# facebookresearch/fast3r

Measured on AMD Instinct MI355X. Metric: views/sec (512^2, ViT-L) single forward pass at N=320, higher is better.
Workload: dtype fp16

## Files before the change

fast3r_amd/csrc/f3r_common.h:

```cpp
#pragma once
#include <hip/hip_runtime.h>
#include <stdint.h>

#include "../../include/f3r.h"

typedef uint32_t u32x4 __attribute__((ext_vector_type(4)));
typedef uint32_t u32x2 __attribute__((ext_vector_type(2)));
typedef _Float16 half8 __attribute__((ext_vector_type(8)));
typedef __bf16 bf8 __attribute__((ext_vector_type(8)));
typedef float float4v __attribute__((ext_vector_type(4)));
typedef float float16v __attribute__((ext_vector_type(16)));

struct F16 {
  typedef _Float16 elem;
  typedef half8 vec8;
  static constexpr int id = F3R_F16;
  static __device__ __forceinline__ float4v mfma16(vec8 a, vec8 b, float4v c) {
    return __builtin_amdgcn_mfma_f32_16x16x32_f16(a, b, c, 0, 0, 0);
  }
  static __device__ __forceinline__ float16v mfma32(vec8 a, vec8 b, float16v c) {
    return __builtin_amdgcn_mfma_f32_32x32x16_f16(a, b, c, 0, 0, 0);
  }
  static __device__ __forceinline__ float16v mfma32k8(u32x2 a, u32x2 b, float16v c) {
    typedef _Float16 h4 __attribute__((ext_vector_type(4)));
    return __builtin_amdgcn_mfma_f32_32x32x8f16(__builtin_bit_cast(h4, a), __builtin_bit_cast(h4, b), c, 0, 0, 0);
  }
  static __device__ __forceinline__ float sum2(uint32_t pk, float acc) {
    typedef _Float16 h2 __attribute__((ext_vector_type(2)));
    const h2 ones = {(_Float16)1.0f, (_Float16)1.0f};
    return __builtin_amdgcn_fdot2(__builtin_bit_cast(h2, pk), ones, acc, false);
  }
};
struct BF16 {
  typedef __bf16 elem;
  typedef bf8 vec8;
  static constexpr int id = F3R_BF16;
  static __device__ __forceinline__ float4v mfma16(vec8 a, vec8 b, float4v c) {
    return __builtin_amdgcn_mfma_f32_16x16x32_bf16(a, b, c, 0, 0, 0);
  }
  static __device__ __forceinline__ float16v mfma32(vec8 a, vec8 b, float16v c) {
    return __builtin_amdgcn_mfma_f32_32x32x16_bf16(a, b, c, 0, 0, 0);
  }
  static __device__ __forceinline__ float16v mfma32k8(u32x2 a, u32x2 b, float16v c) {
    typedef short s4 __attribute__((ext_vector_type(4)));
    return __builtin_amdgcn_mfma_f32_32x32x8bf16_1k(__builtin_bit_cast(s4, a), __builtin_bit_cast(s4, b), c, 0, 0, 0);
  }
  static __device__ __forceinline__ float sum2(uint32_t pk, float acc) {
    typedef __bf16 b2 __attribute__((ext_vector_type(2)));
    const b2 ones = {(__bf16)1.0f, (__bf16)1.0f};
    return __builtin_amdgcn_fdot2_f32_bf16(__builtin_bit_cast(b2, pk), ones, acc, false);
  }
};

template <class T>
__device__ __forceinline__ uint16_t to_lp(float x) {
  typename T::elem e = (typename T::elem)x;
  return __builtin_bit_cast(uint16_t, e);
}
template <class T>
__device__ __forceinline__ uint32_t pack2(float lo, float hi) {
  typedef typename T::elem e2 __attribute__((ext_vector_type(2)));
  e2 p;
  p[0] = (typename T::elem)lo;
  p[1] = (typename T::elem)hi;
  return __builtin_bit_cast(uint32_t, p);
}
template <class T>
__device__ __forceinline__ float from_lp(uint16_t b) {
  return (float)__builtin_bit_cast(typename T::elem, b);
}
template <class T>
__device__ __forceinline__ float lo_f(uint32_t w) { return from_lp<T>((uint16_t)(w & 0xffffu)); }
template <class T>
__device__ __forceinline__ float hi_f(uint32_t w) { return from_lp<T>((uint16_t)(w >> 16)); }

__device__ __forceinline__ uint32_t relu_pk(uint32_t w) {
  uint32_t neg = (w >> 15) & 0x00010001u;
  return w & ~(neg * 0xffffu);
}

template <class T>
__device__ __forceinline__ typename T::vec8 as_vec8(u32x4 v) {
  return __builtin_bit_cast(typename T::vec8, v);
}

bool f3r_gemm256_eligible(const f3r_gemm_args& a);
bool f3r_gemm256_preferred(const f3r_gemm_args& a);
int f3r_gemm256_launch(const f3r_gemm_args& a, hipStream_t stream, int stagger);
int f3r_gemm256_lab(const f3r_gemm_args& a, hipStream_t stream);

bool f3r_gemm_asm_eligible(const f3r_gemm_args& a, const char** why);
bool f3r_gemm_asm_preferred(int64_t tiles);
int f3r_gemm_asm_launch(const f3r_gemm_args& a, hipStream_t stream);
bool f3r_gemm_asm_f8_eligible(const f3r_gemm_args& a, const char** why);
int f3r_gemm_asm_f8_launch(const f3r_gemm_args& a, hipStream_t stream);
bool f3r_gemm_asm_qkv_eligible(const f3r_gemm_args& a, const char** why);
int f3r_gemm_asm_qkv_launch(const f3r_gemm_args& a, hipStream_t stream);

bool f3r_attn_asm_eligible(const f3r_attn_args& a, int64_t min_keys, const char** why);
int f3r_attn_asm_launch(const f3r_attn_args& a, hipStream_t stream);
bool f3r_attn_asm_uses_q256(const f3r_attn_args& a);
bool f3r_attn_asm_splits_tail(const f3r_attn_args& a);

int f3r_attn_generic_launch(const f3r_attn_args& a, hipStream_t stream);

void f3r_set_error(const char* fmt, ...);
int f3r_check_launch(const char* what);

#define F3R_REQUIRE(cond, ...)        \
  do {                                \
    if (!(cond)) {                    \
      f3r_set_error(__VA_ARGS__);     \
      return F3R_ERR_ARG;             \
    }                                 \
  } while (0)
```

fast3r_amd/csrc/f3r_gemm.hip:

```cpp
#include <stdlib.h>

#include "f3r_common.h"
#include "f3r_gemm_epi.h"

namespace {

constexpr int BM = 128, BN = 128, BK = 64, NT = 256;
constexpr int TILE_ELEMS = 128 * 64;
constexpr int GEMM_LDS_BYTES = 2 * 2 * TILE_ELEMS * 2;

__device__ __forceinline__ int swz(int row, int chunk) { return row * 64 + ((chunk ^ ((row >> 1) & 7)) << 3); }

struct ConvRow {
  int b, oy, ox;
  bool ok;
};

template <class T, int A_MODE, int EPI, int GLDS>
__global__ __launch_bounds__(NT, 2) void gemm_kernel(const f3r_gemm_args p) {
  extern __shared__ __attribute__((aligned(16))) uint16_t smem[];
  uint16_t* As = smem;
  uint16_t* Ws = smem + 2 * TILE_ELEMS;

  const int tid = threadIdx.x;
  const int lane = tid & 63;
  const int wid = __builtin_amdgcn_readfirstlane(tid >> 6);
  const int wm = wid >> 1, wn = wid & 1;

  const int n_tiles_n = (p.N + BN - 1) / BN;
  const int64_t n_tiles_m = (p.M + BM - 1) / BM;
  const int64_t n_wg = n_tiles_m * n_tiles_n;
  int64_t wg = blockIdx.x;
  {
    const int64_t q = n_wg / 8, r = n_wg % 8;
    const int64_t xcd = wg % 8, idx = wg / 8;
    wg = (xcd < r ? xcd * (q + 1) : r * (q + 1) + (xcd - r) * q) + idx;
  }
  constexpr int GM = 8;
  const int64_t per_group = (int64_t)GM * n_tiles_n;
  const int64_t grp = wg / per_group;
  const int64_t first_m = grp * GM;
  const int gm = (int)((n_tiles_m - first_m) < GM ? (n_tiles_m - first_m) : GM);
  const int64_t rem_ = wg - grp * per_group;
  const int tn = (int)(rem_ / gm);
  const int64_t tm = first_m + rem_ % gm;
  const int64_t m0 = tm * BM;
  const int n0 = tn * BN;

  const int sc = tid & 7;
  const int sr0 = tid >> 3;
  const uint16_t* Ag = (const uint16_t*)p.A;
  const uint16_t* Wg = (const uint16_t*)p.W;

  ConvRow cr[4];
  int64_t a_row_off[4];
  bool a_row_ok[4];
  bool w_row_ok[4];
  int64_t w_row_off[4];
#pragma unroll
  for (int i = 0; i < 4; ++i) {
    const int64_t m = m0 + sr0 + 32 * i;
    a_row_ok[i] = m < p.M;
    if (A_MODE == F3R_A_PLAIN) {
      a_row_off[i] = m * p.lda;
    } else {
      const int64_t per_img = (int64_t)p.conv_OH * p.conv_OW;
      const int64_t mm = a_row_ok[i] ? m : 0;
      cr[i].b = (int)(mm / per_img);
      const int rem = (int)(mm % per_img);
      cr[i].oy = rem / p.conv_OW;
      cr[i].ox = rem % p.conv_OW;
      cr[i].ok = a_row_ok[i];
      a_row_off[i] = 0;
    }
    const int n = n0 + sr0 + 32 * i;
    w_row_ok[i] = n < p.N;
    w_row_off[i] = (int64_t)n * p.Kpad;
  }

  const int nseg = p.split == F3R_SPLIT_NONE ? 1 : (p.split == F3R_SPLIT_W2 ? 2 : 3);
  const int Kpad1 = p.split == F3R_SPLIT_NONE ? p.Kpad : p.Kpad / 2;
  const int nk1 = Kpad1 / BK;
  const int nk = nseg * nk1;
  const int cpad_tiles = (A_MODE == F3R_A_CONV3X3) ? ((p.conv_C + 63) / 64) : 1;
  const uint16_t* Alo = (const uint16_t*)p.A_lo;

  u32x4 ra[4], rw[4];
  auto load_tile = [&](int kt_all) {
    const int seg = kt_all / nk1;
    const int kt = kt_all - seg * nk1;
    const uint16_t* Ag = (seg == 2) ? Alo : (const uint16_t*)p.A;
    if (A_MODE == F3R_A_PLAIN) {
      const int k = kt * BK + sc * 8;
      const bool kok = (k + 8) <= p.K;
#pragma unroll
      for (int i = 0; i < 4; ++i) {
        u32x4 v = {0u, 0u, 0u, 0u};
        if (a_row_ok[i] && kok) v = *(const u32x4*)(Ag + a_row_off[i] + k);
        ra[i] = v;
      }
    } else {
      const int tap = kt / cpad_tiles;
      const int ci = (kt - tap * cpad_tiles) * 64 + sc * 8;
      const int dy = tap / 3 - 1, dx = tap % 3 - 1;
      const bool cok = ci < p.conv_C;
#pragma unroll
      for (int i = 0; i < 4; ++i) {
        const int iy = cr[i].oy * p.conv_stride + dy;
        const int ix = cr[i].ox * p.conv_stride + dx;
        u32x4 v = {0u, 0u, 0u, 0u};
        if (cr[i].ok && cok && iy >= 0 && iy < p.conv_H && ix >= 0 && ix < p.conv_W) {
          const int64_t off = (((int64_t)cr[i].b * p.conv_H + iy) * p.conv_W + ix) * p.conv_C + ci;
          v = *(const u32x4*)(Ag + off);
          if (p.a_relu) {
            v[0] = relu_pk(v[0]);
            v[1] = relu_pk(v[1]);
            v[2] = relu_pk(v[2]);
            v[3] = relu_pk(v[3]);
          }
        }
        ra[i] = v;
      }
    }
    const int kw = (seg == 1 ? Kpad1 : 0) + kt * BK + sc * 8;
#pragma unroll
    for (int i = 0; i < 4; ++i) {
      u32x4 v = {0u, 0u, 0u, 0u};
      if (w_row_ok[i]) v = *(const u32x4*)(Wg + w_row_off[i] + kw);
      rw[i] = v;
    }
  };
  auto store_tile = [&](int buf) {
    uint16_t* a = As + buf * TILE_ELEMS;
    uint16_t* w = Ws + buf * TILE_ELEMS;
#pragma unroll
    for (int i = 0; i < 4; ++i) {
      const int r = sr0 + 32 * i;
      *(u32x4*)(a + swz(r, sc)) = ra[i];
      *(u32x4*)(w + swz(r, sc)) = rw[i];
    }
  };

  float4v acc[4][4];
#pragma unroll
  for (int i = 0; i < 4; ++i)
#pragma unroll
    for (int j = 0; j < 4; ++j) acc[i][j] = float4v{0.f, 0.f, 0.f, 0.f};

  const int Dq_ = p.qkv_dq ? p.qkv_dq : p.N / 3;
  const bool swap_roles = (EPI == F3R_EPI_QKV) && (n0 + wn * 64 >= Dq_ + (p.N - Dq_) / 2);

  const int fr = lane & 15;
  const int fg = lane >> 4;

  const int offA = (swap_roles ? 0 : 2 * TILE_ELEMS);
  const int offB = (swap_roles ? 2 * TILE_ELEMS : 0);
  const int rowA = (swap_roles ? wm : wn) * 64 + fr;
  const int rowB = (swap_roles ? wn : wm) * 64 + fr;

  auto compute = [&](int buf) {
    const uint16_t* ta = smem + offA + buf * TILE_ELEMS;
    const uint16_t* tb = smem + offB + buf * TILE_ELEMS;
#pragma unroll
    for (int ks = 0; ks < 2; ++ks) {
      typename T::vec8 fa[4], fb[4];
#pragma unroll
      for (int f = 0; f < 4; ++f) {
        fa[f] = as_vec8<T>(*(const u32x4*)(ta + swz(rowA + f * 16, ks * 4 + fg)));
        fb[f] = as_vec8<T>(*(const u32x4*)(tb + swz(rowB + f * 16, ks * 4 + fg)));
      }
#pragma unroll
      for (int i = 0; i < 4; ++i)
#pragma unroll
        for (int j = 0; j < 4; ++j) acc[i][j] = T::mfma16(fa[i], fb[j], acc[i][j]);
    }
  };

  if constexpr (GLDS == 1) {
    typedef __attribute__((address_space(3))) void* lds_ptr_t;
    typedef const __attribute__((address_space(1))) void* glb_ptr_t;
    const int lrow = lane >> 3, pch = lane & 7;
    const uint16_t* asrc[4];
    const uint16_t* wsrc[4];
#pragma unroll
    for (int i = 0; i < 4; ++i) {
      const int r = (wid * 4 + i) * 8 + lrow;
      const int lch = pch ^ ((r >> 1) & 7);
      int64_t m = m0 + r;
      if (m >= p.M) m = p.M - 1;
      int n = n0 + r;
      if (n >= p.N) n = p.N - 1;
      asrc[i] = Ag + m * p.lda + lch * 8;
      wsrc[i] = Wg + (int64_t)n * p.Kpad + lch * 8;
    }
    const int64_t alo_delta = Alo ? (Alo - Ag) : 0;
    auto dma_tile = [&](int kt_all, int buf) {
      const int seg = kt_all / nk1;
      const int kt = kt_all - seg * nk1;
      const int64_t ka = (seg == 2 ? alo_delta : 0) + (int64_t)kt * BK;
      const int kw = (seg == 1 ? Kpad1 : 0) + kt * BK;
#pragma unroll
      for (int i = 0; i < 4; ++i) {
        uint16_t* la = As + buf * TILE_ELEMS + (wid * 4 + i) * 8 * 64;
        uint16_t* lw = Ws + buf * TILE_ELEMS + (wid * 4 + i) * 8 * 64;
        __builtin_amdgcn_global_load_lds((glb_ptr_t)(asrc[i] + ka), (lds_ptr_t)la, 16, 0, 0);
        __builtin_amdgcn_global_load_lds((glb_ptr_t)(wsrc[i] + kw), (lds_ptr_t)lw, 16, 0, 0);
      }
    };
    dma_tile(0, 0);
    __syncthreads();
    int cur = 0;
    for (int kt = 0; kt < nk; ++kt) {
      if (kt + 1 < nk) dma_tile(kt + 1, cur ^ 1);
      compute(cur);
      __syncthreads();
      cur ^= 1;
    }
  } else {
    load_tile(0);
    store_tile(0);
    __syncthreads();
    int cur = 0;
    for (int kt = 0; kt < nk; ++kt) {
      const bool more = (kt + 1) < nk;
      if (more) load_tile(kt + 1);
      compute(cur);
      if (more) store_tile(cur ^ 1);
      __syncthreads();
      cur ^= 1;
    }
  }

  const int64_t m_base = m0 + wm * 64;
  const int n_base = n0 + wn * 64;
  if (swap_roles) gemm_epilogue_vt<T, GemmFragLayout<4, 4, 4, 4>, true>(p, &acc[0][0], m_base, n_base, lane);
  else gemm_epilogue_default<T, EPI, GemmFragLayout<4, 4, 4, 4>, true>(p, &acc[0][0], m_base, n_base, lane);
}

template <class T, int A_MODE, int EPI, int GLDS>
int launch(const f3r_gemm_args& a, hipStream_t stream) {
  static bool attr_set = false;
  auto kern = gemm_kernel<T, A_MODE, EPI, GLDS>;
  if (!attr_set) {
    (void)hipFuncSetAttribute((const void*)kern, hipFuncAttributeMaxDynamicSharedMemorySize, GEMM_LDS_BYTES);
    attr_set = true;
  }
  const int64_t tiles = ((a.M + BM - 1) / BM) * ((a.N + BN - 1) / BN);
  if (tiles <= 0) return F3R_OK;
  F3R_REQUIRE(tiles < (1ll << 31), "f3r_gemm: grid too large");
  hipLaunchKernelGGL(kern, dim3((unsigned)tiles), dim3(NT), GEMM_LDS_BYTES, stream, a);
  return f3r_check_launch("f3r_gemm");
}

template <class T>
int dispatch(const f3r_gemm_args& a, hipStream_t stream) {
  if (a.a_mode == F3R_A_CONV3X3) return launch<T, F3R_A_CONV3X3, F3R_EPI_GENERIC, 0>(a, stream);
  const int Kpad1 = a.split ? a.Kpad / 2 : a.Kpad;
  const bool glds = a.K == Kpad1 && a.M > 0;
  switch (a.epi) {
    case F3R_EPI_GENERIC: return glds ? launch<T, F3R_A_PLAIN, F3R_EPI_GENERIC, 1>(a, stream) : launch<T, F3R_A_PLAIN, F3R_EPI_GENERIC, 0>(a, stream);
    case F3R_EPI_QKV: return glds ? launch<T, F3R_A_PLAIN, F3R_EPI_QKV, 1>(a, stream) : launch<T, F3R_A_PLAIN, F3R_EPI_QKV, 0>(a, stream);
    case F3R_EPI_CONVT: return launch<T, F3R_A_PLAIN, F3R_EPI_CONVT, 0>(a, stream);
  }
  f3r_set_error("f3r_gemm: bad epi %d", a.epi);
  return F3R_ERR_ARG;
}

inline bool al16(const void* p) { return (((uintptr_t)p) & 15) == 0; }
inline bool al8(const void* p) { return (((uintptr_t)p) & 7) == 0; }

}

extern "C" int f3r_gemm(const f3r_gemm_args* args, f3r_stream_t stream) {
  F3R_REQUIRE(args != nullptr, "f3r_gemm: null args");
  const f3r_gemm_args& a = *args;
  F3R_REQUIRE(a.A && a.W, "f3r_gemm: null operand");
  F3R_REQUIRE(a.M >= 0 && a.N > 0, "f3r_gemm: bad M/N (%lld, %d)", (long long)a.M, a.N);
  F3R_REQUIRE(a.split >= F3R_SPLIT_NONE && a.split <= F3R_SPLIT_X3F8, "f3r_gemm: bad split %d", a.split);
  if (a.split == F3R_SPLIT_W2F8) {
    F3R_REQUIRE(al16(a.A) && al16(a.W) && a.w_scale && (((uintptr_t)a.w_scale) & 3) == 0, "f3r_gemm: W2F8 needs 16-byte aligned A / W and w_scale");
    F3R_REQUIRE(a.K > 0 && a.K % 128 == 0 && a.Kpad == a.K, "f3r_gemm: W2F8 needs K = Kpad, a multiple of 128 (got %d / %d)", a.K, a.Kpad);
    F3R_REQUIRE(a.lda % 8 == 0 && a.lda * 2 >= (int64_t)a.K * 3, "f3r_gemm: W2F8 rows are [K fp16 | K fp8]: lda %lld must be >= 3 K / 2", (long long)a.lda);
    F3R_REQUIRE(a.epi != F3R_EPI_GENERIC || a.out_f32 || a.out_lp, "f3r_gemm: no output");
    F3R_REQUIRE(!a.out_f8 && !a.out_relu_f8 && !a.fin_w, "f3r_gemm: W2F8 launches write one output (no out_f8 / out_relu_f8 / fin_w)");
    F3R_REQUIRE((a.kernel_sel >= 0 && a.kernel_sel <= 7) || a.kernel_sel == 9, "f3r_gemm: bad kernel_sel %d", a.kernel_sel);
    F3R_REQUIRE(a.dtype == F3R_F16, "f3r_gemm: W2F8 corrects fp16 planes only (dtype %d)", a.dtype);
    F3R_REQUIRE(a.act >= F3R_ACT_NONE && a.act <= F3R_ACT_RELU, "f3r_gemm: bad act %d", a.act);
    F3R_REQUIRE(a.N % 4 == 0 && (!a.bias || al16(a.bias)), "f3r_gemm: N %d must be a multiple of 4, bias 16-byte aligned", a.N);
    if (a.epi == F3R_EPI_GENERIC) {
      F3R_REQUIRE(!a.out_f32 || (al16(a.out_f32) && a.ldo_f32 % 4 == 0 && a.ldo_f32 >= a.N), "f3r_gemm: out_f32 alignment/ld");
      F3R_REQUIRE(!a.out_lp || (al16(a.out_lp) && a.ldo_lp % 8 == 0 && a.ldo_lp >= a.N), "f3r_gemm: out_lp alignment/ld");
      F3R_REQUIRE(!a.res_f32 || (al16(a.res_f32) && a.ldr_f32 % 4 == 0 && a.ldr_f32 >= a.N), "f3r_gemm: res_f32 alignment/ld");
    }
    const char* why = "";
    if (a.epi == F3R_EPI_QKV) {
      F3R_REQUIRE(a.qkv_dq != 0 || a.N % 3 == 0, "f3r_gemm: QKV with three equal parts needs N %% 3 == 0 (got %d)", a.N);
      {
        const int Dq = a.qkv_dq ? a.qkv_dq : a.N / 3;
        F3R_REQUIRE(Dq > 0 && Dq % 64 == 0 && a.N > Dq && (a.N - Dq) % 128 == 0, "f3r_gemm: QKV parts must be whole 64-wide heads (N %d, q %d)", a.N, Dq);
      }
      F3R_REQUIRE(a.q && a.k && a.vt && a.W_aux && al16(a.W_aux) && a.seq_len > 0 && a.M % a.seq_len == 0 && a.ldvt >= a.seq_len && a.act == F3R_ACT_NONE,
                  "f3r_gemm: W2F8 QKV needs q, k, vt, W_aux (16-byte aligned), seq_len dividing M, no activation");
      if (a.rope_cos) F3R_REQUIRE(a.rope_sin && a.rope_w > 0 && al16(a.rope_cos) && al16(a.rope_sin), "f3r_gemm: RoPE tables");
      if (!f3r_gemm_asm_qkv_eligible(a, &why)) {
        f3r_set_error("f3r_gemm: split W2F8 QKV but the launch is not eligible for the hand-scheduled kernel: %s", why);
        return F3R_ERR_UNSUPPORTED;
      }
      return f3r_gemm_asm_qkv_launch(a, (hipStream_t)stream);
    }
    if (!f3r_gemm_asm_f8_eligible(a, &why)) {
      f3r_set_error("f3r_gemm: split W2F8 (fp8 low plane) but the launch is not eligible for the hand-scheduled kernel: %s", why);
      return F3R_ERR_UNSUPPORTED;
    }
    return f3r_gemm_asm_f8_launch(a, (hipStream_t)stream);
  }
  F3R_REQUIRE(a.epi == F3R_EPI_GENERIC || (!a.out_f8 && !a.out_relu_f8 && !a.fin_w), "f3r_gemm: out_f8 / out_relu_f8 / fin_w need the generic epilogue (epi %d)", a.epi);
  const int planes = a.split ? 2 : 1;
  F3R_REQUIRE(a.Kpad > 0 && a.Kpad % (64 * planes) == 0, "f3r_gemm: Kpad %d must be a positive multiple of %d", a.Kpad, 64 * planes);
  const int Kpad1 = a.Kpad / planes;
  F3R_REQUIRE((a.split != F3R_SPLIT_X3 && a.split != F3R_SPLIT_X3F8) || (a.A_lo && al16(a.A_lo) && !a.a_relu), "f3r_gemm: X3 / X3F8 split needs A_lo (16-byte aligned) and no a_relu");
  if (a.split == F3R_SPLIT_X3F8)
    F3R_REQUIRE(a.a_mode == F3R_A_CONV3X3 && a.dtype == F3R_F16 && a.conv_C % 128 == 0 && a.w_scale && (((uintptr_t)a.w_scale) & 3) == 0,
                "f3r_gemm: X3F8 needs a 3x3 convolution with conv_C %% 128 == 0 (got %d), fp16 planes and w_scale", a.conv_C);
  F3R_REQUIRE((a.kernel_sel >= 0 && a.kernel_sel <= 7) || a.kernel_sel == 9 || a.kernel_sel >= 16, "f3r_gemm: bad kernel_sel %d", a.kernel_sel);
  F3R_REQUIRE(a.N % 4 == 0, "f3r_gemm: N %d must be a multiple of 4", a.N);
  F3R_REQUIRE(al16(a.A) && al16(a.W), "f3r_gemm: A/W must be 16-byte aligned");
  F3R_REQUIRE(a.dtype == F3R_F16 || a.dtype == F3R_BF16, "f3r_gemm: bad dtype %d", a.dtype);
  if (a.a_mode == F3R_A_PLAIN) {
    F3R_REQUIRE(a.K > 0 && a.K % 8 == 0 && a.K <= Kpad1, "f3r_gemm: K %d must be a multiple of 8 and <= Kpad", a.K);
    F3R_REQUIRE(a.lda % 8 == 0 && a.lda >= a.K, "f3r_gemm: lda %lld must be a multiple of 8 and >= K", (long long)a.lda);
  } else if (a.a_mode == F3R_A_CONV3X3) {
    F3R_REQUIRE(a.conv_C > 0 && a.conv_C % 8 == 0, "f3r_gemm: conv_C %d must be a multiple of 8", a.conv_C);
    F3R_REQUIRE(Kpad1 == 9 * ((a.conv_C + 63) / 64) * 64, "f3r_gemm: conv Kpad %d != 9*roundup(C,64) per plane", a.Kpad);
    F3R_REQUIRE(a.epi == F3R_EPI_GENERIC, "f3r_gemm: conv3x3 supports only the generic epilogue");
    F3R_REQUIRE(a.conv_stride == 1 || a.conv_stride == 2, "f3r_gemm: conv stride %d", a.conv_stride);
    F3R_REQUIRE(a.conv_OH == (a.conv_H + 2 - 3) / a.conv_stride + 1 && a.conv_OW == (a.conv_W + 2 - 3) / a.conv_stride + 1,
                "f3r_gemm: conv output dims inconsistent");
    F3R_REQUIRE(a.conv_OH > 0 && a.conv_OW > 0 && a.M % ((int64_t)a.conv_OH * a.conv_OW) == 0, "f3r_gemm: conv M not a multiple of OH*OW");
  } else {
    f3r_set_error("f3r_gemm: bad a_mode %d", a.a_mode);
    return F3R_ERR_ARG;
  }
  if (a.epi == F3R_EPI_GENERIC) {
    F3R_REQUIRE(a.out_f32 || a.out_lp || a.fin_w, "f3r_gemm: no output");
    F3R_REQUIRE(!a.out_f32 || (al16(a.out_f32) && a.ldo_f32 % 4 == 0 && a.ldo_f32 >= a.N), "f3r_gemm: out_f32 alignment/ld");
    F3R_REQUIRE(!a.out_lp || (al8(a.out_lp) && a.ldo_lp % 4 == 0 && a.ldo_lp >= a.N), "f3r_gemm: out_lp alignment/ld");
    F3R_REQUIRE((!a.out_f8 && !a.out_relu_f8) || (a.dtype == F3R_F16 && a.N % 8 == 0 && al8(a.out_f8) && al8(a.out_relu_f8) && !a.out_lp_f8),
                "f3r_gemm: out_f8 / out_relu_f8 need fp16, N %% 8 == 0 and 8-byte aligned buffers");
    if (a.fin_w) {
      F3R_REQUIRE(a.fin_b && a.fin_pts && al16(a.fin_w) && (a.fin_n_out == 3 || a.fin_n_out == 4) && (a.fin_n_out == 4 || !a.fin_conf),
                  "f3r_gemm: fin_w needs fin_b, fin_pts, a 16-byte aligned [4][N] weight and fin_n_out 3 or 4 (a confidence output needs 4)");
      F3R_REQUIRE(a.fin_depth_mode >= 0 && a.fin_depth_mode <= 2 && (a.fin_conf_mode == 0 || a.fin_conf_mode == 1), "f3r_gemm: bad fin_depth_mode / fin_conf_mode");
      F3R_REQUIRE(!a.out_f32 && !a.out_relu && !a.out_f8 && !a.out_relu_f8 && !a.res_lp && !a.res_f32 && !a.rowadd,
                  "f3r_gemm: the fused head tail writes fin_pts / fin_conf only");
    }
    F3R_REQUIRE(!a.res_f32 || (al16(a.res_f32) && a.ldr_f32 % 4 == 0), "f3r_gemm: res_f32 alignment/ld");
    F3R_REQUIRE(!a.res_lp || (al8(a.res_lp) && a.ldr_lp % 4 == 0), "f3r_gemm: res_lp alignment/ld");
    F3R_REQUIRE(!a.res_lp2 || (al8(a.res_lp2) && a.ldr_lp2 % 4 == 0), "f3r_gemm: res_lp2 alignment/ld");
    F3R_REQUIRE((!a.res_lp_lo || (a.res_lp && al8(a.res_lp_lo))) && (!a.res_lp2_lo || (a.res_lp2 && al8(a.res_lp2_lo))), "f3r_gemm: low residual planes need their high planes");
    F3R_REQUIRE((!a.out_lp_lo || (a.out_lp && al8(a.out_lp_lo))) && (!a.out_relu || (al8(a.out_relu) && a.ldo_lp % 4 == 0 && a.ldo_lp >= a.N)) &&
                (!a.out_relu_lo || (a.out_relu && al8(a.out_relu_lo))), "f3r_gemm: out_lp_lo / out_relu alignment");
    F3R_REQUIRE(!a.rowadd || (al16(a.rowadd) && a.rowadd_div > 0), "f3r_gemm: rowadd alignment/div");
    const int64_t ld_max = 1ll << 26;
    F3R_REQUIRE((!a.out_f32 || a.ldo_f32 < ld_max) && (!a.out_lp || a.ldo_lp < ld_max) && (!a.res_f32 || (a.ldr_f32 >= 0 && a.ldr_f32 < ld_max)) &&
                (!a.res_lp || (a.ldr_lp >= 0 && a.ldr_lp < ld_max)) && (!a.res_lp2 || (a.ldr_lp2 >= 0 && a.ldr_lp2 < ld_max)), "f3r_gemm: row strides must be < 2^26 elements");
    F3R_REQUIRE(!a.bias || al16(a.bias), "f3r_gemm: bias alignment");
  } else if (a.epi == F3R_EPI_QKV) {
    const int Dq = a.qkv_dq ? a.qkv_dq : a.N / 3;
    F3R_REQUIRE(a.qkv_dq != 0 || a.N % 3 == 0, "f3r_gemm: QKV with three equal parts needs N %% 3 == 0 (got %d)", a.N);
    F3R_REQUIRE(Dq > 0 && Dq % 64 == 0 && a.N > Dq && (a.N - Dq) % 128 == 0, "f3r_gemm: QKV parts must be whole 64-wide heads (N %d, q %d)", a.N, Dq);
    F3R_REQUIRE(a.q && a.k && a.vt && al8(a.q) && al8(a.k) && al8(a.vt), "f3r_gemm: QKV outputs null/misaligned");
    F3R_REQUIRE(a.seq_len > 0 && a.M % a.seq_len == 0 && a.ldvt >= a.seq_len, "f3r_gemm: QKV seq_len/ldvt");
    F3R_REQUIRE(a.act == F3R_ACT_NONE, "f3r_gemm: QKV has no activation");
    F3R_REQUIRE(!a.bias || al16(a.bias), "f3r_gemm: bias alignment");
    if (a.rope_cos) F3R_REQUIRE(a.rope_sin && a.rope_w > 0 && al16(a.rope_cos) && al16(a.rope_sin), "f3r_gemm: RoPE tables");
  } else if (a.epi == F3R_EPI_CONVT) {
    F3R_REQUIRE(a.out_lp && al8(a.out_lp), "f3r_gemm: CONVT needs out_lp");
    F3R_REQUIRE(a.ct_s > 0 && a.ct_cout > 0 && a.ct_cout % 4 == 0 && a.N == a.ct_s * a.ct_s * a.ct_cout, "f3r_gemm: CONVT N != s*s*cout");
    F3R_REQUIRE(a.ct_h > 0 && a.ct_w > 0 && a.M % ((int64_t)a.ct_h * a.ct_w) == 0, "f3r_gemm: CONVT M not a multiple of h*w");
    F3R_REQUIRE(!a.bias || al16(a.bias), "f3r_gemm: bias alignment");
  }
  hipStream_t s = (hipStream_t)stream;
  if (a.kernel_sel >= 16) return f3r_gemm256_lab(a, s);
  if (a.split == F3R_SPLIT_X3F8 || a.fin_w) {
    if (!f3r_gemm256_eligible(a)) {
      f3r_set_error("f3r_gemm: split X3F8 / fin_w but the launch is not eligible for the 256-tile kernel (conv_C %% 64 (X3F8: 128) == 0, "
                    "N %% 128 == 0 (fin_w: N == 128), operand below 4 GiB)");
      return F3R_ERR_UNSUPPORTED;
    }
    return f3r_gemm256_launch(a, s, 1);
  }
  if (a.kernel_sel == 6 || a.kernel_sel == 0 || a.kernel_sel == 9) {
    const char* why = "";
    if (a.epi == F3R_EPI_QKV && f3r_gemm_asm_qkv_eligible(a, &why) && (a.kernel_sel == 6 || a.kernel_sel == 9 || f3r_gemm_asm_preferred((a.M / 256) * (a.N / 3 / 256))))
      return f3r_gemm_asm_qkv_launch(a, s);
    const bool ok = a.epi != F3R_EPI_QKV && f3r_gemm_asm_eligible(a, &why);
    if ((a.kernel_sel == 6 || a.kernel_sel == 9) && !ok) {
      f3r_set_error("f3r_gemm: kernel_sel 6 (hand-scheduled kernel) but the launch is not eligible: %s", why);
      return F3R_ERR_UNSUPPORTED;
    }
    if (ok && (a.kernel_sel == 6 || a.kernel_sel == 9 || f3r_gemm_asm_preferred((a.M / 256) * (a.N / 256)))) return f3r_gemm_asm_launch(a, s);
  }
  const int sel = a.kernel_sel == 7 ? 0 : a.kernel_sel;
  if (sel >= 2) F3R_REQUIRE(f3r_gemm256_eligible(a), "f3r_gemm: kernel_sel %d but the shape is not eligible for the 256-tile kernel", sel);
  if (sel >= 2 || (sel == 0 && f3r_gemm256_eligible(a) && f3r_gemm256_preferred(a))) return f3r_gemm256_launch(a, s, sel != 3);
  return a.dtype == F3R_F16 ? dispatch<F16>(a, s) : dispatch<BF16>(a, s);
}
```

fast3r_amd/csrc/f3r_gemm256.hip:

```cpp
#include "f3r_gemm256_impl.h"

int f3r_gemm256_run_bf16(const f3r_gemm_args& a, hipStream_t stream, int stagger);
int f3r_gemm256_run_conv_f8_fin(const f3r_gemm_args& a, hipStream_t stream);

bool f3r_gemm256_eligible(const f3r_gemm_args& a) {
  if (a.N % 128 != 0) return false;
  if (a.epi == F3R_EPI_QKV) {
    const int Dq = a.qkv_dq ? a.qkv_dq : a.N / 3;
    if (Dq % 256 != 0 || ((a.N - Dq) / 2) % 256 != 0) return false;
  }
  const int Kpad1 = a.split ? a.Kpad / 2 : a.Kpad;
  if (Kpad1 % 64 != 0) return false;
  if (a.a_mode == F3R_A_PLAIN) {
    if (a.K != Kpad1) return false;
    if ((int64_t)256 * a.lda * 2 >= (1ll << 32)) return false;
  } else {
    if (a.a_relu || a.conv_C % 64 != 0) return false;
    if (a.M / ((int64_t)a.conv_OH * a.conv_OW) * a.conv_H * a.conv_W * a.conv_C * 2 >= (1ll << 32)) return false;
    if (a.split == F3R_SPLIT_X3F8 && (a.conv_C % 128 != 0 || a.dtype != F3R_F16)) return false;
  }
  if (a.split == F3R_SPLIT_X3F8 && a.a_mode != F3R_A_CONV3X3) return false;
  if (a.fin_w && (a.a_mode != F3R_A_CONV3X3 || a.N != 128 || a.epi != F3R_EPI_GENERIC)) return false;
  if ((int64_t)256 * a.Kpad * 2 >= (1ll << 32)) return false;
  const int add = gemm_additive_pattern(a);
  if (add == F3R_ADD_UNSUPPORTED || (add != F3R_ADD_NONE && a.act != F3R_ACT_NONE)) return false;
  if (add != F3R_ADD_NONE && a.epi != F3R_EPI_GENERIC) return false;
  if (a.a_mode == F3R_A_CONV3X3 ? (add == F3R_ADD_RES_F32 || add == F3R_ADD_ROWADD) : add == F3R_ADD_RES_LP) return false;
  return true;
}

bool f3r_gemm256_preferred(const f3r_gemm_args& a) { return score_256(a, tile_halves(a)) >= score_128(a); }

int f3r_gemm256_launch(const f3r_gemm_args& a, hipStream_t stream, int stagger) {
  const int64_t tiles = ((a.M + BM - 1) / BM) * ((a.N + 127) / 128);
  if (tiles <= 0) return F3R_OK;
  F3R_REQUIRE(tiles < (1ll << 31), "f3r_gemm: grid too large");
  if (a.split == F3R_SPLIT_X3F8 || a.fin_w) return f3r_gemm256_run_conv_f8_fin(a, stream);
  return a.dtype == F3R_F16 ? dispatch256<F16>(a, stream, stagger) : f3r_gemm256_run_bf16(a, stream, stagger);
}
```

fast3r_amd/csrc/f3r_gemm256_f8.hip:

```cpp
#include <cstdlib>

#include "f3r_gemm256_impl.h"

int f3r_gemm256_run_conv_f8_fin(const f3r_gemm_args& a, hipStream_t stream) {
  const bool f8 = a.split == F3R_SPLIT_X3F8;
  const int add = gemm_additive_pattern(a);
  if (a.fin_w) {
#ifdef F3R_CONV_ABLATIONS
    if (f8) {
      static const char* ab = getenv("F3R_CONV_ABLATE");
      switch (ab ? atoi(ab) : 0) {
#define F3R_ABL(n) case n: return launch256<F16, F3R_A_CONV3X3, F3R_EPI_GENERIC, 1, F3R_ADD_NONE, 1, true, true, false, n>(a, stream);
        F3R_ABL(1) F3R_ABL(1024) F3R_ABL(2048) F3R_ABL(2) F3R_ABL(4) F3R_ABL(3) F3R_ABL(7)
#undef F3R_ABL
      }
    }
#endif
    if (a.dtype == F3R_BF16) return launch256<BF16, F3R_A_CONV3X3, F3R_EPI_GENERIC, 1, F3R_ADD_NONE, 1, false, true>(a, stream);
    if (f8 && a.kernel_sel == 5) return launch256<F16, F3R_A_CONV3X3, F3R_EPI_GENERIC, 1, F3R_ADD_NONE, 1, true, true, true>(a, stream);
    return f8 ? launch256<F16, F3R_A_CONV3X3, F3R_EPI_GENERIC, 1, F3R_ADD_NONE, 1, true, true>(a, stream)
              : launch256<F16, F3R_A_CONV3X3, F3R_EPI_GENERIC, 1, F3R_ADD_NONE, 1, false, true>(a, stream);
  }
  const int nh = tile_halves(a);
  if (add == F3R_ADD_RES_LP)
    return nh == 2 ? launch256<F16, F3R_A_CONV3X3, F3R_EPI_GENERIC, 1, F3R_ADD_RES_LP, 2, true>(a, stream)
                   : launch256<F16, F3R_A_CONV3X3, F3R_EPI_GENERIC, 1, F3R_ADD_RES_LP, 1, true>(a, stream);
  return nh == 2 ? launch256<F16, F3R_A_CONV3X3, F3R_EPI_GENERIC, 1, F3R_ADD_NONE, 2, true>(a, stream)
                 : launch256<F16, F3R_A_CONV3X3, F3R_EPI_GENERIC, 1, F3R_ADD_NONE, 1, true>(a, stream);
}
```

Measured before the change: 35.87.

## Add strip-staged persistent 3x3 conv kernel for X3F8 split convolutions

Adds a persistent conv kernel for the X3F8 fp16+fp8 3x3 convolution. It loads a contiguous 264-row strip of input pixels into LDS once per (dy, channel-tile) and reuses it across the three dx taps by shifting the fragment read address. Image-edge columns are handled by redirecting reads to zeroed LDS blocks rather than reloading the operand per tap. It also prefetches the next tile's operands before the epilogue. By default it is chosen when kernel_sel is 0 and the launch is the fused head tail (fin_w) or has N not a multiple of 256. This trades per-tap global/LDS traffic for more LDS, a single workgroup per CU, and extra complexity in edge masking.

```diff
diff --git a/fast3r_amd/csrc/f3r_common.h b/fast3r_amd/csrc/f3r_common.h
--- a/fast3r_amd/csrc/f3r_common.h
+++ b/fast3r_amd/csrc/f3r_common.h
@@ -86,6 +86,7 @@
 
 bool f3r_gemm256_eligible(const f3r_gemm_args& a);
 bool f3r_gemm256_preferred(const f3r_gemm_args& a);
+bool f3r_conv_strip_eligible(const f3r_gemm_args& a);
 int f3r_gemm256_launch(const f3r_gemm_args& a, hipStream_t stream, int stagger);
 int f3r_gemm256_lab(const f3r_gemm_args& a, hipStream_t stream);
 
diff --git a/fast3r_amd/csrc/f3r_conv_strip.h b/fast3r_amd/csrc/f3r_conv_strip.h
--- /dev/null
+++ b/fast3r_amd/csrc/f3r_conv_strip.h
@@ -0,0 +1,98 @@
+#pragma once
+#include <cstdint>
+
+#if defined(__HIPCC__) || defined(__CUDACC__)
+#define F3R_HD __host__ __device__ inline
+#else
+#define F3R_HD inline
+#endif
+
+namespace f3r_strip {
+
+constexpr int TILE_ROWS = 256;
+constexpr int STRIP_ROWS = 264;
+constexpr int ROW_BYTES = 128;
+constexpr int PIECE_ROWS = 8;
+constexpr int PIECES_PER_WAVE = 4;
+constexpr int SLOT_BYTES = 34 * 1024;
+constexpr int ZERO_BYTES = 8 * 1024;
+constexpr int SLOT_STRIDE = SLOT_BYTES + ZERO_BYTES;
+constexpr int N_SLOTS = 2;
+constexpr int W_SLOT_BYTES = 16 * 1024;
+constexpr int N_W_SLOTS = 3;
+constexpr int W_BASE = N_SLOTS * SLOT_STRIDE;
+constexpr int FIN_BASE = W_BASE + N_W_SLOTS * W_SLOT_BYTES;
+constexpr int FIN_BYTES = 16 * 1024;
+constexpr int TAB_BASE = FIN_BASE + FIN_BYTES;
+constexpr int TAB_ENTRIES = 512;
+constexpr int LDS_BYTES = TAB_BASE + TAB_ENTRIES * 16;
+static_assert(LDS_BYTES <= 160 * 1024, "LDS map");
+static_assert(SLOT_BYTES % 2048 == 0 && SLOT_STRIDE % 2048 == 0, "zero blocks must be 2 KiB-aligned");
+
+struct KTile {
+  int seg;
+  int dy;
+  int ct;
+  int dx;
+};
+F3R_HD int nk1_of(int C) { return 9 * (C / 64); }
+F3R_HD int nk8_of(int C) { return 9 * (C / 128); }
+F3R_HD int nk_of(int C) { return nk1_of(C) + 2 * nk8_of(C); }
+F3R_HD KTile ktile(int t, int C) {
+  KTile k;
+  int u = t, cts = C / 64;
+  k.seg = 0;
+  if (t >= nk1_of(C)) {
+    u = t - nk1_of(C);
+    cts = C / 128;
+    k.seg = 1 + u / nk8_of(C);
+    u -= (k.seg - 1) * nk8_of(C);
+  }
+  k.dx = u % 3;
+  u /= 3;
+  k.ct = u % cts;
+  k.dy = u / cts;
+  return k;
+}
+F3R_HD uint32_t w_soff(const KTile& k, int C) {
+  const int tap = k.dy * 3 + k.dx, Kpad1 = 9 * C;
+  if (k.seg == 0) return (uint32_t)((tap * (C / 64) + k.ct) * 64 * 2);
+  return (uint32_t)((k.seg + 1) * Kpad1 + (tap * (C / 128) + k.ct) * 128);
+}
+F3R_HD int32_t a_delta(const KTile& k, int W, int C) {
+  return (k.dy - 1) * W * 2 * C + k.ct * 128 + (k.seg == 2 ? C : 0);
+}
+F3R_HD bool a_plane_f8(const KTile& k) { return k.seg != 0; }
+
+F3R_HD int piece_of(int wave, int i) { return i < PIECES_PER_WAVE ? wave * PIECES_PER_WAVE + i : 32; }
+F3R_HD int strip_row_of_lane(int wave, int i, int lane) { return piece_of(wave, i) * PIECE_ROWS + (lane >> 3); }
+F3R_HD int swz_key(int row) { return row & 6; }
+F3R_HD int src_chunk_of_lane(int row, int lane) { return (lane & 7) ^ swz_key(row); }
+F3R_HD uint32_t lds_addr_of_lane(int slot, int wave, int i, int lane) {
+  return (uint32_t)(slot * SLOT_STRIDE + piece_of(wave, i) * PIECE_ROWS * ROW_BYTES + lane * 16);
+}
+F3R_HD uint32_t strip_src_off(int64_t img_pix0, int p0, int s, int chunk, int C) {
+  return (uint32_t)((img_pix0 + p0 - 1 + s) * (int64_t)(2 * C) + chunk * 16);
+}
+F3R_HD bool strip_row_valid(int p0, int s, int dy, int W, int HW) {
+  const int r = p0 - 1 + s + (dy - 1) * W;
+  return s < TILE_ROWS + 2 && r >= 0 && r < HW;
+}
+
+F3R_HD int frag_strip_row(int j, int dx) { return j + dx; }
+F3R_HD uint32_t frag_addr(int slot, int row, int chunk) { return (uint32_t)(slot * SLOT_STRIDE + row * ROW_BYTES + ((chunk ^ swz_key(row)) << 4)); }
+F3R_HD bool frag_is_pad(int p, int dx, int W) {
+  const int x = p % W;
+  return (dx == 0 && x == 0) || (dx == 2 && x == W - 1);
+}
+F3R_HD uint32_t zero_addr(int slot, uint32_t addr, int mf) { return (uint32_t)(slot * SLOT_STRIDE + SLOT_BYTES + mf * 2048) + (addr & 2047u); }
+
+F3R_HD bool shape_eligible(int H, int W, int C, int stride, int OH, int OW) {
+  if (stride != 1 || OH != H || OW != W) return false;
+  if (C <= 0 || C % 128 != 0) return false;
+  if ((int64_t)OH * OW % TILE_ROWS != 0) return false;
+  if (nk_of(C) > TAB_ENTRIES) return false;
+  return true;
+}
+
+}
diff --git a/fast3r_amd/csrc/f3r_conv_strip.hip b/fast3r_amd/csrc/f3r_conv_strip.hip
--- /dev/null
+++ b/fast3r_amd/csrc/f3r_conv_strip.hip
@@ -0,0 +1,16 @@
+#include "f3r_conv_strip_impl.h"
+
+bool f3r_conv_strip_eligible(const f3r_gemm_args& a) {
+  if (a.a_mode != F3R_A_CONV3X3 || a.split != F3R_SPLIT_X3F8 || a.dtype != F3R_F16 || a.N % 128 != 0) return false;
+  if (!f3r_strip::shape_eligible(a.conv_H, a.conv_W, a.conv_C, a.conv_stride, a.conv_OH, a.conv_OW)) return false;
+  if (a.Kpad != 2 * 9 * a.conv_C || a.M % 256 != 0) return false;
+  if (a.fin_w) return true;
+  f3r_gemm_args b = a;
+  b.kernel_sel = 0;
+  return tile_halves(b) == 1;
+}
+
+int f3r_conv_strip_run(const f3r_gemm_args& a, hipStream_t stream) {
+  if (a.fin_w) return launch_conv_strip<F3R_ADD_NONE, true>(a, stream);
+  return gemm_additive_pattern(a) == F3R_ADD_RES_LP ? launch_conv_strip<F3R_ADD_RES_LP, false>(a, stream) : launch_conv_strip<F3R_ADD_NONE, false>(a, stream);
+}
diff --git a/fast3r_amd/csrc/f3r_conv_strip_impl.h b/fast3r_amd/csrc/f3r_conv_strip_impl.h
--- /dev/null
+++ b/fast3r_amd/csrc/f3r_conv_strip_impl.h
@@ -0,0 +1,339 @@
+#pragma once
+#include "f3r_conv_strip.h"
+#include "f3r_gemm256_impl.h"
+
+namespace {
+
+typedef __attribute__((address_space(3))) char* lds_bytes_t;
+typedef __attribute__((address_space(3))) u32x4* lds_u32x4_t;
+
+template <int ADDSRC, bool FIN>
+__device__ __forceinline__ void conv_strip_body(const f3r_gemm_args& p, const lds_bytes_t smem, const int64_t m0_tile, const int n0_tile, const bool first,
+                                                const bool has_next, const int64_t m0_next, const int n0_next) {
+  namespace S = f3r_strip;
+  typedef F16 T;
+  constexpr bool PAIRED = true;
+  static_assert(ADDSRC == F3R_ADD_NONE || ADDSRC == F3R_ADD_RES_LP, "convolutions take lowp residuals only");
+  static_assert(!FIN || ADDSRC == F3R_ADD_NONE, "fused head tail: no additive terms");
+  const int tid = threadIdx.x;
+  const int lane = tid & 63;
+  const int wid = __builtin_amdgcn_readfirstlane(tid >> 6);
+  const int wm = wid >> 2, wn = wid & 3;
+  const int fr = lane & 15, fg = lane >> 4;
+  auto w_key = [](int r) { return ((r >> 1) & 1) | (((r >> 3) & 3) << 1); };
+
+  const int C = p.conv_C, CW = p.conv_W, HW = p.conv_H * p.conv_W;
+  const int nk1 = S::nk1_of(C), nk8 = S::nk8_of(C), nk = nk1 + 2 * nk8;
+  const int G16 = nk1 / 3, G8 = nk8 / 3, G = G16 + 2 * G8;
+
+  const char* const Ab = (const char*)p.A;
+  const char* const Alo = (const char*)p.A_lo;
+  const uint32_t a_bytes = (uint32_t)(p.M / HW * HW * C * 2);
+  const char* Wb = nullptr;
+  uint32_t wsc[2];
+  uint32_t w_off[2];
+  uint32_t s_off[5];
+  uint32_t s_msk[5];
+  uint32_t zmask = 0;
+  auto setup_tile = [&](int64_t tm0, int tn0) {
+    Wb = (const char*)p.W + (int64_t)tn0 * p.Kpad * 2;
+#pragma unroll
+    for (int nf = 0; nf < 2; ++nf) {
+      int n = tn0 + wn * 32 + (fr >> 2) * 8 + (fr & 3) + nf * 4;
+      if (n >= p.N) n = p.N - 1;
+      wsc[nf] = p.w_scale[n];
+    }
+#pragma unroll
+    for (int i = 0; i < 2; ++i) {
+      const int r = (wid * 2 + i) * 8 + (lane >> 3);
+      int n = tn0 + r;
+      if (n >= p.N) n = p.N - 1;
+      w_off[i] = (uint32_t)(((int64_t)(n - tn0) * p.Kpad + ((lane & 7) ^ w_key(r)) * 8) * 2);
+    }
+    const int64_t img = tm0 / HW;
+    const int p0 = (int)(tm0 - img * HW);
+#pragma unroll
+    for (int i = 0; i < 5; ++i) {
+      const int s = S::strip_row_of_lane(wid, i, lane);
+      s_off[i] = S::strip_src_off(img * HW, p0, s, S::src_chunk_of_lane(s, lane), C);
+      uint32_t msk = 0;
+#pragma unroll
+      for (int dy = 0; dy < 3; ++dy)
+        if (!S::strip_row_valid(p0, s, dy, CW, HW)) msk |= 1u << dy;
+      s_msk[i] = msk;
+    }
+    zmask = 0;
+    const int x0 = (p0 + wm * 64 + fr) % CW;
+#pragma unroll
+    for (int q = 0; q < 8; ++q) {
+      const int x = (x0 + (q >> 2) * 128 + (q & 3) * 16) % CW;
+      if (x == 0) zmask |= 1u << q;
+      if (x == CW - 1) zmask |= 1u << (8 + q);
+    }
+  };
+  setup_tile(m0_tile, n0_tile);
+
+  const lds_bytes_t tab = smem + S::TAB_BASE;
+  if (first) {
+    for (int t = tid; t < nk; t += NT) {
+      const S::KTile k = S::ktile(t, C);
+      *(lds_u32x4_t)(tab + t * 16) = u32x4{(uint32_t)S::a_delta(k, CW, C), (uint32_t)(k.dy | (S::a_plane_f8(k) ? 16 : 0)), S::w_soff(k, C), 0u};
+    }
+#pragma unroll
+    for (int s = 0; s < S::N_SLOTS; ++s)
+      *(lds_u32x4_t)(smem + s * S::SLOT_STRIDE + S::SLOT_BYTES + tid * 16) = u32x4{0u, 0u, 0u, 0u};
+    __syncthreads();
+  }
+  u32x4 ea = {0u, 0u, 0u, 0u}, ew = ea;
+  int a_g = 0, w_t = 0;
+  auto fetch_a = [&]() { ea = *(lds_u32x4_t)(tab + a_g * 48); };
+  auto fetch_w = [&]() { ew = *(lds_u32x4_t)(tab + w_t * 16); };
+  auto a_advance = [&]() { if (a_g + 1 < G) ++a_g; };
+  auto w_advance = [&]() { if (w_t + 1 < nk) ++w_t; };
+  auto issue_strip = [&](int slot, int i0, int n, bool halo) {
+    const int a_delta = __builtin_amdgcn_readfirstlane((int)ea[0]);
+    const int meta = __builtin_amdgcn_readfirstlane((int)ea[1]);
+    const int dy = meta & 3;
+    const __amdgpu_buffer_rsrc_t rs = __builtin_amdgcn_make_buffer_rsrc((void*)((meta & 16) ? Alo : Ab), 0, a_bytes, 0x00020000);
+    const lds_bytes_t dst = smem + slot * S::SLOT_STRIDE;
+    auto one = [&](int i, int piece) {
+      const int32_t inv = ((int32_t)(s_msk[i] << (31 - dy))) >> 31;
+      const uint32_t vo = (s_off[i] + (uint32_t)a_delta) | (uint32_t)inv;
+      __builtin_amdgcn_raw_ptr_buffer_load_lds(rs, (lds_ptr_t)(dst + piece * 1024), 16, (int)vo, 0, 0, 0);
+    };
+    if (halo && wid == 0) one(4, 32);
+#pragma unroll
+    for (int i = 0; i < 4; ++i)
+      if (i >= i0 && i < i0 + n) one(i, wid * S::PIECES_PER_WAVE + i);
+  };
+  auto issue_w = [&](int slot) {
+    const int w_soff = __builtin_amdgcn_readfirstlane((int)ew[2]);
+    const __amdgpu_buffer_rsrc_t rs = __builtin_amdgcn_make_buffer_rsrc((void*)Wb, 0, 0x7fffffff, 0x00020000);
+    const lds_bytes_t dst = smem + S::W_BASE + slot * S::W_SLOT_BYTES + wid * 2048;
+#pragma unroll
+    for (int i = 0; i < 2; ++i) __builtin_amdgcn_raw_ptr_buffer_load_lds(rs, (lds_ptr_t)(dst + i * 1024), 16, (int)w_off[i], w_soff, 0, 0);
+  };
+
+  int a_rd[3][2][2], z_rd[3][2], w_rd[2];
+  const int w_row = wn * 32 + (fr >> 2) * 8 + (fr & 3);
+#pragma unroll
+  for (int ks = 0; ks < 2; ++ks) {
+#pragma unroll
+    for (int dx = 0; dx < 3; ++dx) {
+#pragma unroll
+      for (int h = 0; h < 2; ++h) a_rd[dx][ks][h] = (int)S::frag_addr(0, S::frag_strip_row(h * 128 + wm * 64 + fr, dx), ks * 4 + fg);
+      z_rd[dx][ks] = (int)S::zero_addr(0, (uint32_t)a_rd[dx][ks][0], 0);
+    }
+    w_rd[ks] = S::W_BASE + w_row * 128 + (((ks * 4 + fg) ^ w_key(w_row)) << 4);
+  }
+
+  float4v acc[16];
+  typename T::vec8 fa0[2][4], fa1[2][4], fw[2][2];
+  typedef uint32_t u32x8 __attribute__((ext_vector_type(8)));
+  typedef int i32x8 __attribute__((ext_vector_type(8)));
+  u32x8 ga0[4], ga1[4], gw[2];
+
+  auto read_a = [&](auto e8, auto which, auto slc, auto dxc) {
+    constexpr int h = decltype(which)::value, SL = decltype(slc)::value, DX = decltype(dxc)::value;
+    uint32_t zm = zmask;
+    if constexpr (DX != 1) asm volatile("" : "+v"(zm));
+#pragma unroll
+    for (int mf = 0; mf < 4; ++mf) {
+      int r0 = a_rd[DX][0][h], r1 = a_rd[DX][1][h];
+      if constexpr (DX != 1) {
+        const bool pad = (zm >> ((DX == 2 ? 8 : 0) + h * 4 + mf)) & 1u;
+        r0 = pad ? z_rd[DX][0] : r0;
+        r1 = pad ? z_rd[DX][1] : r1;
+      }
+      const u32x4 c0 = *(lds_u32x4_t)(smem + r0 + SL * S::SLOT_STRIDE + mf * 2048);
+      const u32x4 c1 = *(lds_u32x4_t)(smem + r1 + SL * S::SLOT_STRIDE + mf * 2048);
+      if constexpr (decltype(e8)::value) {
+        (h ? ga1 : ga0)[mf] = __builtin_shufflevector(c0, c1, 0, 1, 2, 3, 4, 5, 6, 7);
+      } else {
+        (h ? fa1 : fa0)[0][mf] = as_vec8<T>(c0);
+        (h ? fa1 : fa0)[1][mf] = as_vec8<T>(c1);
+      }
+    }
+  };
+  auto read_w = [&](auto e8, int slot) {
+#pragma unroll
+    for (int nf = 0; nf < 2; ++nf) {
+      const u32x4 c0 = *(lds_u32x4_t)(smem + w_rd[0] + slot * S::W_SLOT_BYTES + nf * 4 * 128);
+      const u32x4 c1 = *(lds_u32x4_t)(smem + w_rd[1] + slot * S::W_SLOT_BYTES + nf * 4 * 128);
+      if constexpr (decltype(e8)::value) {
+        gw[nf] = __builtin_shufflevector(c0, c1, 0, 1, 2, 3, 4, 5, 6, 7);
+      } else {
+        fw[0][nf] = as_vec8<T>(c0);
+        fw[1][nf] = as_vec8<T>(c1);
+      }
+    }
+  };
+  auto mma = [&](auto e8, auto which, int sa_shift, int sb) {
+    constexpr int mh = decltype(which)::value;
+    if constexpr (decltype(e8)::value) {
+      auto& g = mh ? ga1 : ga0;
+#pragma unroll
+      for (int nf = 0; nf < 2; ++nf) {
+        const int sa = (int)((wsc[nf] >> sa_shift) & 0xffu);
+#pragma unroll
+        for (int mf = 0; mf < 4; ++mf)
+          acc[nf * 8 + mh * 4 + mf] = __builtin_amdgcn_mfma_scale_f32_16x16x128_f8f6f4(__builtin_bit_cast(i32x8, gw[nf]), __builtin_bit_cast(i32x8, g[mf]),
+                                                                                      acc[nf * 8 + mh * 4 + mf], 0, 0, 0, sa, 0, sb);
+      }
+#pragma unroll
+      for (int nf = 0; nf < 2; ++nf)
+#pragma unroll
+        for (int mf = 0; mf < 4; ++mf) asm volatile("" : "+v"(acc[nf * 8 + mh * 4 + mf]));
+    } else {
+      auto& f = mh ? fa1 : fa0;
+#pragma unroll
+      for (int ks = 0; ks < 2; ++ks)
+#pragma unroll
+        for (int nf = 0; nf < 2; ++nf)
+#pragma unroll
+          for (int mf = 0; mf < 4; ++mf) acc[nf * 8 + mh * 4 + mf] = T::mfma16(fw[ks][nf], f[ks][mf], acc[nf * 8 + mh * 4 + mf]);
+    }
+  };
+
+#define F3R_STRIP_MMA(WHICH)                 \
+  __builtin_amdgcn_sched_barrier(0);         \
+  __builtin_amdgcn_s_barrier();              \
+  F3R_LGKMCNT0();                            \
+  __builtin_amdgcn_sched_barrier(0);         \
+  __builtin_amdgcn_s_setprio(1);             \
+  mma(e8, IC<WHICH>{}, sa_shift, sb);        \
+  __builtin_amdgcn_s_setprio(0);             \
+  __builtin_amdgcn_sched_barrier(0);         \
+  __builtin_amdgcn_s_barrier();
+  auto ktile = [&](auto dxc, auto slc, auto e8, int sa_shift, int sb) {
+    constexpr int DX = decltype(dxc)::value, SL = decltype(slc)::value;
+    fetch_w();
+    read_w(e8, DX);
+    __builtin_amdgcn_sched_barrier(0);
+    read_a(e8, IC<0>{}, slc, dxc);
+    issue_w((DX + 2) % 3);
+    w_advance();
+    F3R_STRIP_MMA(0)
+    if constexpr (DX < 2) fetch_a();
+    read_a(e8, IC<1>{}, slc, dxc);
+    if constexpr (DX == 0) {
+      issue_strip(SL ^ 1, 0, 2, true);
+      F3R_VMCNT(4);
+    } else if constexpr (DX == 1) {
+      issue_strip(SL ^ 1, 2, 2, false);
+      a_advance();
+      F3R_VMCNT(6);
+    } else {
+      F3R_VMCNT(2);
+    }
+    F3R_STRIP_MMA(1)
+  };
+#undef F3R_STRIP_MMA
+  auto group = [&](auto slc, auto e8, int sa_shift, int sb) {
+    ktile(IC<0>{}, slc, e8, sa_shift, sb);
+    ktile(IC<1>{}, slc, e8, sa_shift, sb);
+    ktile(IC<2>{}, slc, e8, sa_shift, sb);
+  };
+
+  typedef GemmFragLayout<2, 8, 2, 4, PAIRED> Frag;
+  const int64_t m_base = m0_tile + wm * 64;
+  const int n_base = n0_tile + wn * 32;
+  auto opening_loads = [&](bool issue) {
+    a_g = w_t = 0;
+    if (issue) {
+      fetch_a();
+      fetch_w();
+      issue_strip(0, 0, 4, true);
+      issue_w(0);
+    }
+    a_advance();
+    w_advance();
+    if (issue) {
+      fetch_w();
+      issue_w(1);
+    }
+    w_advance();
+  };
+  opening_loads(first);
+  gemm_acc_init_additive<T, Frag, ADDSRC, false>(p, acc, m_base, n_base, lane);
+  F3R_VMCNT(0);
+  __builtin_amdgcn_s_barrier();
+  if (wm == 1) __builtin_amdgcn_s_barrier();
+
+  typedef IC<0> E16;
+  typedef IC<1> E8;
+  for (int g = 0; g < G16; g += 2) {
+    group(IC<0>{}, E16{}, 0, 0);
+    group(IC<1>{}, E16{}, 0, 0);
+  }
+  for (int g = 0; g < 2 * G8; g += 2) {
+    group(IC<0>{}, E8{}, g >= G8 ? 8 : 0, g >= G8 ? 115 : 127);
+    group(IC<1>{}, E8{}, g + 1 >= G8 ? 8 : 0, g + 1 >= G8 ? 115 : 127);
+  }
+  F3R_VMCNT(0);
+  if (wm == 0) __builtin_amdgcn_s_barrier();
+  if (has_next) {
+    setup_tile(m0_next, n0_next);
+    opening_loads(true);
+  }
+
+  if constexpr (FIN) {
+    __builtin_amdgcn_s_barrier();
+    gemm_epilogue_fin<T, Frag>(p, acc, m0_tile, wm, wn, lane, tid, (float*)(smem + S::FIN_BASE));
+  } else {
+    gemm_epilogue_default<T, F3R_EPI_GENERIC, Frag, false>(p, acc, m_base, n_base, lane);
+  }
+}
+
+template <int ADDSRC, bool FIN>
+__global__ __launch_bounds__(NT, 1) void conv_strip_kernel(const f3r_gemm_args p) {
+  extern __shared__ __attribute__((aligned(2048))) char smem_strip[];
+  constexpr int BN = 128;
+  const int n_tiles_n = (p.N + BN - 1) / BN;
+  const int64_t n_tiles_m = p.M / BM;
+  const int64_t n_wg = n_tiles_m * n_tiles_n;
+  auto tile_of = [&](int64_t wg, int64_t& m0, int& n0) {
+    {
+      const int64_t q = n_wg / 8, r = n_wg % 8;
+      const int64_t xcd = wg % 8, idx = wg / 8;
+      wg = (xcd < r ? xcd * (q + 1) : r * (q + 1) + (xcd - r) * q) + idx;
+    }
+    constexpr int GM = 8;
+    const int64_t per_group = (int64_t)GM * n_tiles_n;
+    const int64_t grp = wg / per_group;
+    const int64_t first_m = grp * GM;
+    const int gm = (int)((n_tiles_m - first_m) < GM ? (n_tiles_m - first_m) : GM);
+    const int64_t rem_ = wg - grp * per_group;
+    const int tn = (int)(rem_ / gm);
+    const int64_t tm = first_m + rem_ % gm;
+    m0 = tm * BM;
+    n0 = tn * BN;
+  };
+  int64_t m0, m0n = 0;
+  int n0, n0n = 0;
+  bool first = true;
+  for (int64_t v = blockIdx.x; v < n_wg; v += gridDim.x) {
+    tile_of(v, m0, n0);
+    const bool has_next = v + gridDim.x < n_wg;
+    if (has_next) tile_of(v + gridDim.x, m0n, n0n);
+    conv_strip_body<ADDSRC, FIN>(p, (lds_bytes_t)smem_strip, m0, n0, first, has_next, m0n, n0n);
+    first = false;
+  }
+}
+
+template <int ADDSRC, bool FIN>
+int launch_conv_strip(const f3r_gemm_args& a, hipStream_t stream) {
+  static bool attr_set = false;
+  auto kern = conv_strip_kernel<ADDSRC, FIN>;
+  constexpr int LDS_BYTES = f3r_strip::LDS_BYTES;
+  if (!attr_set) {
+    (void)hipFuncSetAttribute((const void*)kern, hipFuncAttributeMaxDynamicSharedMemorySize, LDS_BYTES);
+    attr_set = true;
+  }
+  const int64_t tiles = (a.M / BM) * ((a.N + 127) / 128);
+  const int64_t grid = tiles <= f3r_num_cus() ? tiles : f3r_num_cus();
+  hipLaunchKernelGGL(kern, dim3((unsigned)grid), dim3(NT), LDS_BYTES, stream, a);
+  return f3r_check_launch("f3r_gemm(conv strip)");
+}
+
+}
diff --git a/fast3r_amd/csrc/f3r_gemm.hip b/fast3r_amd/csrc/f3r_gemm.hip
--- a/fast3r_amd/csrc/f3r_gemm.hip
+++ b/fast3r_amd/csrc/f3r_gemm.hip
@@ -322,7 +322,8 @@
   if (a.split == F3R_SPLIT_X3F8)
     F3R_REQUIRE(a.a_mode == F3R_A_CONV3X3 && a.dtype == F3R_F16 && a.conv_C % 128 == 0 && a.w_scale && (((uintptr_t)a.w_scale) & 3) == 0,
                 "f3r_gemm: X3F8 needs a 3x3 convolution with conv_C %% 128 == 0 (got %d), fp16 planes and w_scale", a.conv_C);
-  F3R_REQUIRE((a.kernel_sel >= 0 && a.kernel_sel <= 7) || a.kernel_sel == 9 || a.kernel_sel >= 16, "f3r_gemm: bad kernel_sel %d", a.kernel_sel);
+  F3R_REQUIRE((a.kernel_sel >= 0 && a.kernel_sel <= 7) || (a.kernel_sel >= 9 && a.kernel_sel <= 11) || a.kernel_sel >= 16, "f3r_gemm: bad kernel_sel %d", a.kernel_sel);
+  F3R_REQUIRE((a.kernel_sel != 10 && a.kernel_sel != 11) || a.split == F3R_SPLIT_X3F8, "f3r_gemm: kernel_sel %d names a form of the X3F8 convolution", a.kernel_sel);
   F3R_REQUIRE(a.N % 4 == 0, "f3r_gemm: N %d must be a multiple of 4", a.N);
   F3R_REQUIRE(al16(a.A) && al16(a.W), "f3r_gemm: A/W must be 16-byte aligned");
   F3R_REQUIRE(a.dtype == F3R_F16 || a.dtype == F3R_BF16, "f3r_gemm: bad dtype %d", a.dtype);
@@ -388,6 +389,10 @@
                     "N %% 128 == 0 (fin_w: N == 128), operand below 4 GiB)");
       return F3R_ERR_UNSUPPORTED;
     }
+    if (a.kernel_sel == 11 && !f3r_conv_strip_eligible(a)) {
+      f3r_set_error("f3r_gemm: kernel_sel 11 (strip form) but the launch is not eligible: stride 1, conv_OH * conv_OW %% 256 == 0, the 256 x 128 tile form");
+      return F3R_ERR_UNSUPPORTED;
+    }
     return f3r_gemm256_launch(a, s, 1);
   }
   if (a.kernel_sel == 6 || a.kernel_sel == 0 || a.kernel_sel == 9) {
diff --git a/fast3r_amd/csrc/f3r_gemm256.hip b/fast3r_amd/csrc/f3r_gemm256.hip
--- a/fast3r_amd/csrc/f3r_gemm256.hip
+++ b/fast3r_amd/csrc/f3r_gemm256.hip
@@ -22,6 +22,11 @@
   if (a.split == F3R_SPLIT_X3F8 && a.a_mode != F3R_A_CONV3X3) return false;
   if (a.fin_w && (a.a_mode != F3R_A_CONV3X3 || a.N != 128 || a.epi != F3R_EPI_GENERIC)) return false;
   if ((int64_t)256 * a.Kpad * 2 >= (1ll << 32)) return false;
+  if (a.a_mode == F3R_A_CONV3X3) {
+    const int nk1 = Kpad1 / 64;
+    const int nk = a.split == F3R_SPLIT_X3F8 ? 2 * nk1 : (a.split == F3R_SPLIT_NONE ? 1 : (a.split == F3R_SPLIT_W2 ? 2 : 3)) * nk1;
+    if (nk > TileCfg<2>::TAB_ENTRIES) return false;
+  }
   const int add = gemm_additive_pattern(a);
   if (add == F3R_ADD_UNSUPPORTED || (add != F3R_ADD_NONE && a.act != F3R_ACT_NONE)) return false;
   if (add != F3R_ADD_NONE && a.epi != F3R_EPI_GENERIC) return false;
diff --git a/fast3r_amd/csrc/f3r_gemm256_f8.hip b/fast3r_amd/csrc/f3r_gemm256_f8.hip
--- a/fast3r_amd/csrc/f3r_gemm256_f8.hip
+++ b/fast3r_amd/csrc/f3r_gemm256_f8.hip
@@ -2,9 +2,13 @@
 
 #include "f3r_gemm256_impl.h"
 
+bool f3r_conv_strip_eligible(const f3r_gemm_args& a);
+int f3r_conv_strip_run(const f3r_gemm_args& a, hipStream_t stream);
+
 int f3r_gemm256_run_conv_f8_fin(const f3r_gemm_args& a, hipStream_t stream) {
   const bool f8 = a.split == F3R_SPLIT_X3F8;
   const int add = gemm_additive_pattern(a);
+  if (a.kernel_sel == 11 || (a.kernel_sel == 0 && (a.fin_w || a.N % 256 != 0) && f3r_conv_strip_eligible(a))) return f3r_conv_strip_run(a, stream);
   if (a.fin_w) {
 #ifdef F3R_CONV_ABLATIONS
     if (f8) {
```

Result: no change. 35.89 (median of 4 runs) (+0.1%).
